# Mephisto405/WCMC

Measured on AMD Instinct MI355X. Metric: 128x128 MC patches/sec (train step), KPCN-Manifold, higher is better.
Workload: dtype bf16x321h

## Files before the change

### wcmc_amd/csrc/conv_bf16x3.hip

```cpp
#include <stdlib.h>

#include "common.h"
#include "conv_common.h"

namespace wcmc {

typedef __bf16 bf16x8 __attribute__((ext_vector_type(8)));
typedef unsigned short u16;
typedef short s16x4 __attribute__((ext_vector_type(4)));

__device__ __forceinline__ u16 f2bf(float x) { return __builtin_bit_cast(u16, (__bf16)x); }
__device__ __forceinline__ float bf2f(u16 h) { return __builtin_bit_cast(float, (unsigned)h << 16); }
__device__ __forceinline__ void split1(float x, u16& hi, u16& lo) {
  hi = f2bf(x);
  lo = f2bf(x - bf2f(hi));
}

__global__ void split_kernel(const float* __restrict__ x, int64_t xsn, int64_t xsh, int64_t xsw,
                             u16* __restrict__ out, int H, int W, int C, int Cp, int64_t total,
                             const float* __restrict__ post = nullptr, int64_t psn = 0, int64_t psh = 0, int64_t psw = 0,
                             int act = 0, float slope = 0.f) {
  const int V = Cp / 8;
  for (int64_t idx = (int64_t)blockIdx.x * blockDim.x + threadIdx.x; idx < total;
       idx += (int64_t)gridDim.x * blockDim.x) {
// ... 2372 lines not shown
  const int g = lane >> 4, li = lane & 15, tq = li >> 2, tp = li & 3;
  const int prow0 = wk * 32 + 4 * g + tq;
  auto tr_read = [&](const u16* base, int stride, int col0, bf16x8& out) {
    const u16* a0 = base + prow0 * stride + col0 + 4 * tp;
    const s16x4 lo4 = __builtin_amdgcn_ds_read_tr16_b64_v4i16(
        (s16x4 __attribute__((address_space(3)))*)(a0));
    const s16x4 hi4 = __builtin_amdgcn_ds_read_tr16_b64_v4i16(
        (s16x4 __attribute__((address_space(3)))*)(a0 + 16 * stride));
    typedef short s16x8 __attribute__((ext_vector_type(8)));
    const s16x8 cat = {lo4[0], lo4[1], lo4[2], lo4[3], hi4[0], hi4[1], hi4[2], hi4[3]};
    out = __builtin_bit_cast(bf16x8, cat);
  };

  if (nstages > 0) load_stage();
  for (int st = 0; st < nstages; ++st) {
    __syncthreads();
    store_stage();
    __syncthreads();
    if (st + 1 < nstages) load_stage();
    bf16x8 xh[4], xl[PL == 2 ? 4 : 1], yh[MT], yl[PL == 2 ? MT : 1];
#pragma unroll
    for (int j = 0; j < 4; ++j) {
      tr_read(Xs, SB, j * 16, xh[j]);
      if constexpr (PL == 2) tr_read(Xs + PK * SB, SB, j * 16, xl[j]);
    }
#pragma unroll
    for (int i = 0; i < MT; ++i) {
      tr_read(Ys, SA, (wm * MT + i) * 16, yh[i]);
      if constexpr (PL == 2) tr_read(Ys + PK * SA, SA, (wm * MT + i) * 16, yl[i]);
    }
    __builtin_amdgcn_sched_barrier(0);
#pragma unroll
    for (int i = 0; i < MT; ++i) {
      if (i < tm_valid) {
#pragma unroll
        for (int j = 0; j < 4; ++j) {
          if (j < tn_valid) {
            if constexpr (PL == 2) {
              acc[i][j] = __builtin_amdgcn_mfma_f32_16x16x32_bf16(yl[i], xh[j], acc[i][j], 0, 0, 0);
              acc[i][j] = __builtin_amdgcn_mfma_f32_16x16x32_bf16(yh[i], xl[j], acc[i][j], 0, 0, 0);
            }
            acc[i][j] = __builtin_amdgcn_mfma_f32_16x16x32_bf16(yh[i], xh[j], acc[i][j], 0, 0, 0);
          }
        }
      }
    }
  }
  __syncthreads();

  constexpr int RS = XC + 4;
  float* red = reinterpret_cast<float*>(smem16);
  const int fcol = lane & 15, fq = (lane >> 4) * 4;
  for (int h = 0; h < 2; ++h) {
    if (wk == h) {
#pragma unroll
      for (int i = 0; i < MT; ++i) {
        if (wm * MT + i < TM) {
#pragma unroll
          for (int j = 0; j < 4; ++j)
#pragma unroll
            for (int r = 0; r < 4; ++r) {
              float* q = red + ((wm * MT + i) * 16 + fq + r) * RS + j * 16 + fcol;
              *q = (h == 0 ? 0.f : *q) + acc[i][j][r];
            }
        }
      }
    }
    __syncthreads();
  }
  float* slab = p.slabs + ((int64_t)s * taps + tap) * p.Np * p.Cq;
  for (int idx = tid; idx < YC * (XC / 4); idx += 256) {
    const int r = idx / (XC / 4), c = (idx - r * (XC / 4)) * 4;
    if (co0 + r < p.Np && ci0 + c < p.Cq)
      *reinterpret_cast<float4*>(slab + (int64_t)(co0 + r) * p.Cq + ci0 + c) =
          *reinterpret_cast<const float4*>(red + r * RS + c);
  }
}


struct XWRowsParams {
  const u16* x; int N, H, W, Cpi;
  const u16* dy; int Ho, Wo, Cpo;
  int pad;
  float* slabs; int S, rps, R;
  float* dbg;
  int prio;
  int Np, Cq, coBlocks, ciBlocks;
  unsigned x_bytes, dy_bytes;
  int xps, yps;
};

constexpr int xwr_stride(int ch) { return ((ch / 16) | 1) * 16; }

struct XwrRaw { u32x2 a, b; };
template <int OFF2>
__device__ __forceinline__ void xwr_tr_issue(unsigned addr, XwrRaw& r) {
  asm volatile("ds_read_b64_tr_b16 %0, %2\n\tds_read_b64_tr_b16 %1, %2 offset:%3" : "=&v"(r.a), "=&v"(r.b) : "v"(addr), "n"(OFF2));
}
__device__ __forceinline__ bf16x8 xwr_cat(const XwrRaw& r) {
  const u32x4 c = {r.a[0], r.a[1], r.b[0], r.b[1]};
  return __builtin_bit_cast(bf16x8, c);
}

template <int OFF1, int OFF2>
__device__ __forceinline__ void xwr_tr_issue_at(unsigned addr, XwrRaw& r) {
  asm volatile("ds_read_b64_tr_b16 %0, %2 offset:%3\n\tds_read_b64_tr_b16 %1, %2 offset:%4"
               : "=&v"(r.a), "=&v"(r.b) : "v"(addr), "n"(OFF1), "n"(OFF2));
}

template <class F, int... I>
__device__ __forceinline__ void xstatic_for_impl(F&& f, std::integer_sequence<int, I...>) { (f(std::integral_constant<int, I>{}), ...); }
template <int N, class F>
__device__ __forceinline__ void xstatic_for(F&& f) { xstatic_for_impl(static_cast<F&&>(f), std::make_integer_sequence<int, N>{}); }

template <int KS, int TM, int NW, int DBG = 0, int PL = 2>
__global__ __launch_bounds__(NW * 64, (NW <= 4 ? 2 : 1)) void conv_wgrad_rows_bf16x3_kernel(XWRowsParams p) {
  constexpr int CHY = TM * 16, CHX = NW * 16, PK = 64, XR = PK + KS - 1;
  constexpr int SY = xwr_stride(CHY), SX = xwr_stride(CHX);
  constexpr int VY = SY / 8, VX = SX / 8;
  constexpr int YV = PK * VY, XV = XR * VX;
  constexpr int NVEC = PL * YV + PL * XV;
  constexpr int NI = (NVEC + NW * 64 - 1) / (NW * 64);
  constexpr int BUF = NI * NW * 64 * 8;
  extern __shared__ __attribute__((aligned(16))) u16 smem16[];

  const int tid = threadIdx.x, lane = tid & 63, wave = __builtin_amdgcn_readfirstlane(tid >> 6);
  const int xcd = blockIdx.x & 7, local = blockIdx.x >> 3;
  const int unit = (local / KS) * 8 + xcd;
  const int upb = p.coBlocks * p.ciBlocks;
  if (unit >= p.S * upb) return;
  const int trow = local % KS;
  const int s = unit / upb, ub = unit - s * upb;
  const int cob = ub / p.ciBlocks, cib = ub - cob * p.ciBlocks;
  const int co0 = cob * CHY, ci0 = cib * CHX;
  const int r0 = s * p.rps, r1 = min(p.R, r0 + p.rps);
  const int nch = (p.Wo + PK - 1) / PK;
  const int nrows = r1 - r0;
  const int nst = nrows * nch;

  const __amdgpu_buffer_rsrc_t xr = __builtin_amdgcn_make_buffer_rsrc((void*)p.x, 0, (int)p.x_bytes, 0x00020000);
  const __amdgpu_buffer_rsrc_t yr = __builtin_amdgcn_make_buffer_rsrc((void*)p.dy, 0, (int)p.dy_bytes, 0x00020000);

  unsigned relv[NI]; int rowv[NI];
#pragma unroll
  for (int i = 0; i < NI; ++i) {
    const int v = (i * NW + wave) * 64 + lane;
    unsigned rel = 0; int rw = 127;
    if (v < PL * YV) {
      const int plane = v >= YV, vv = v - plane * YV;
      const int row = vv / VY, vec = vv - row * VY;
      const int co = co0 + vec * 8;
      if (vec * 8 < CHY && co < p.Cpo) { rel = (unsigned)(row * p.yps + plane * 2 * p.Cpo + co * 2); rw = row; }
    } else if (v < NVEC) {
      const int u = v - PL * YV;
      const int plane = u >= XV, uu = u - plane * XV;
      const int row = uu / VX, vec = uu - row * VX;
      const int ci = ci0 + vec * 8;
      if (vec * 8 < CHX && ci < p.Cpi) { rel = (unsigned)(row * p.xps + plane * 2 * p.Cpi + ci * 2); rw = row; }
    }
    relv[i] = rel; rowv[i] = rw;
  }
  unsigned f_ybase = 0, f_xbase = 0, f_yn = 0, f_xn = 0; int f_xlo = 0, f_buf = 0;
  int f_c = 0, f_rs = nrows > 0 ? (nrows - trow % nrows) % nrows : 0, f_n, f_oy;
  const int f_n0 = r0 / p.Ho, f_oy0 = r0 - f_n0 * p.Ho;
  { const int r = r0 + f_rs; f_n = r / p.Ho; f_oy = r - f_n * p.Ho; }
  auto issue_prep = [&](int buf) {
// ... 475 lines not shown
                acc[q][i] = __builtin_amdgcn_mfma_f32_16x16x32_bf16(yh, xl[q], acc[q][i], 0, 0, 0);
              }
              acc[q][i] = __builtin_amdgcn_mfma_f32_16x16x32_bf16(yh, xh[q], acc[q][i], 0, 0, 0);
            }
            if (i == TM - 1 && kk + 1 < nk) {
              constexpr int K1 = 32 * SX * 2;
              XWR8_READ(K1, K1 + 16 * SX * 2, ax[q], rxh[q]);
              if constexpr (PL == 2) XWR8_READ(K1 + XLO, K1 + XLO + 16 * SX * 2, ax[q], rxl[q]);
            }
          }
          if (fill && kk * TM + i == 0) issue_prep(par ^ 1);
          if (fill && kk * TM + i < NI) issue_one(kk * TM + i);
          __builtin_amdgcn_sched_barrier(0);
        }
      }
    }
    if (fill) {
#pragma unroll
      for (int i = 0; i < NI; ++i)
        if (i >= nk * TM) issue_one(i);
    }
    cst(2);
  };
  for (int st = 0; st < nst; st += 2) {
    stage(st, std::integral_constant<int, 0>{});
    if (st + 1 < nst) stage(st + 1, std::integral_constant<int, 1>{});
  }
  rts(2);

  __syncthreads();
  constexpr int RS = CHX + 4;
  float* red = reinterpret_cast<float*>(smem16);
  const int fcol = lane & 15, fq = (lane >> 4) * 4;
  int etap[NS], eci[NS];
#pragma unroll
  for (int q = 0; q < NS; ++q) { const int pr = NS * wave + q; etap[q] = pr / NCI; eci[q] = pr - etap[q] * NCI; }
#pragma unroll
  for (int t = 0; t < KS; ++t) {
#pragma unroll
    for (int q = 0; q < NS; ++q)
      if (etap[q] == t) {
#pragma unroll
        for (int i = 0; i < TM; ++i)
#pragma unroll
          for (int r = 0; r < 4; ++r) red[(ycol[i] * 16 + fq + r) * RS + eci[q] * 16 + fcol] = acc[q][i][r];
      }
    if (XE) {
      if (t == ETAP) {
#pragma unroll
        for (int j = 0; j < NA; ++j)
          if (j < nex) {
#pragma unroll
            for (int r = 0; r < 4; ++r) red[(ycol[j] * 16 + fq + r) * RS + (ECI0 + epair) * 16 + fcol] = ace[j][r];
          }
      }
    } else if (t == ETAP && wave < TM) {
#pragma unroll
      for (int e = 0; e < NF; ++e)
#pragma unroll
        for (int r = 0; r < 4; ++r) red[(wave * 16 + fq + r) * RS + (ECI0 + e) * 16 + fcol] = ace[e][r];
    }
    __syncthreads();
    float* slab = p.slabs + (((int64_t)s * KS * KS + trow * KS + t) * p.Np + co0) * p.Cq + ci0;
    for (int idx = tid; idx < CHY * (CHX / 4); idx += NW * 64) {
      const int row = idx / (CHX / 4), v = idx - row * (CHX / 4);
      if (co0 + row < p.Np && ci0 + v * 4 < p.Cq)
        *reinterpret_cast<float4*>(slab + (int64_t)row * p.Cq + v * 4) = *reinterpret_cast<const float4*>(red + row * RS + v * 4);
    }
    __syncthreads();
  }
  if (DBG & 16) {
    asm volatile("s_waitcnt vmcnt(0)" ::: "memory");
    rts(3);
    if (lane == 0) {
      unsigned long long* o = reinterpret_cast<unsigned long long*>(p.dbg) + ((int64_t)blockIdx.x * NW + wave) * 8;
      for (int i = 0; i < 4; ++i) o[i] = rt[i];
      for (int i = 0; i < 3; ++i) o[4 + i] = cyc[i];
      o[7] = (unsigned long long)nst;
    }
  }
}
#undef XWR8_READ

template <int KS, int TM, int NW, int PL = 2>
static constexpr size_t xwr_lds_bytes() {
  constexpr int NVEC = PL * 64 * (xwr_stride(TM * 16) / 8) + PL * (64 + KS - 1) * (xwr_stride(NW * 16) / 8);
  constexpr int NI = (NVEC + NW * 64 - 1) / (NW * 64);
  constexpr size_t stage = (size_t)2 * NI * NW * 64 * 16;
  constexpr size_t red = (size_t)TM * 16 * (NW * 16 + 4) * sizeof(float);
  return stage > red ? stage : red;
}
static size_t xwr_lds_bytes_rt(int ks, int tm, int nw, int pl = 2) {
  const int nvec = pl * 64 * (xwr_stride(tm * 16) / 8) + pl * (64 + ks - 1) * (xwr_stride(nw * 16) / 8);
  const int ni = (nvec + nw * 64 - 1) / (nw * 64);
  const size_t stage = (size_t)2 * ni * nw * 64 * 16, red = (size_t)tm * 16 * (nw * 16 + 4) * sizeof(float);
  return stage > red ? stage : red;
}

template <int KS, int TM, int NW, int PL = 2>
static int launch_xwgrad_rows(const XWRowsParams& q, hipStream_t st) {
  constexpr size_t lds = xwr_lds_bytes<KS, TM, NW, PL>();
  const dim3 grid((unsigned)(((q.S * q.coBlocks * q.ciBlocks + 7) / 8) * 8 * KS));
  const char* r8e = ab_env("WCMC_WGRAD_ROWS8");
  const bool rows8 = r8e ? r8e[0] != '0' : PL == 2;
  if (KS == 5 && TM == 7 && NW == 7 && rows8) {
    constexpr size_t lds8 = (size_t)2 * ((PL * (64 * 14 + 68 * 14) + 511) / 512) * 512 * 16;
    if (PL == 1) {
      static LdsAttr attr81_set;
      if (set_max_lds(reinterpret_cast<const void*>(&conv_wgrad_rows8_bf16x3_kernel<0, 1, 1>), (size_t)lds8, attr81_set) != hipSuccess) return WCMC_ERR_LAUNCH;
      hipLaunchKernelGGL((conv_wgrad_rows8_bf16x3_kernel<0, 1, 1>), grid, dim3(512), lds8, st, q);
      return check_launch("conv2d_wgrad_bf16x3(rows8, one plane)");
    }
    static LdsAttr attr8_set, attr80_set;
#ifdef WCMC_DEBUG_BUILD
    { const char* e = ab_env("WCMC_DEBUG_ABLATE");
      const int ab = e ? atoi(e) : 0;
      auto kfn = ab == 16 ? &conv_wgrad_rows8_bf16x3_kernel<16> : ab == 1 ? &conv_wgrad_rows8_bf16x3_kernel<1> : ab == 2 ? &conv_wgrad_rows8_bf16x3_kernel<2>
                 : ab == 3 ? &conv_wgrad_rows8_bf16x3_kernel<3> : ab == 8 ? &conv_wgrad_rows8_bf16x3_kernel<8> : ab == 32 ? &conv_wgrad_rows8_bf16x3_kernel<32>
                 : ab == 34 ? &conv_wgrad_rows8_bf16x3_kernel<34> : ab == 35 ? &conv_wgrad_rows8_bf16x3_kernel<35> : nullptr;
      if (kfn) {
        (void)hipFuncSetAttribute(reinterpret_cast<const void*>(kfn), hipFuncAttributeMaxDynamicSharedMemorySize, (int)lds8);
        hipLaunchKernelGGL(kfn, grid, dim3(512), lds8, st, q);
        return check_launch("conv2d_wgrad_bf16x3(rows8 ablation / stamps)");
      } }
#endif
    if (set_max_lds(reinterpret_cast<const void*>(&conv_wgrad_rows8_bf16x3_kernel<0, 1>), (size_t)lds8, attr8_set) != hipSuccess) return WCMC_ERR_LAUNCH;
    if (set_max_lds(reinterpret_cast<const void*>(&conv_wgrad_rows8_bf16x3_kernel<0, 0>), (size_t)lds8, attr80_set) != hipSuccess) return WCMC_ERR_LAUNCH;
    if (x_env_on("WCMC_WGRAD_ROWS8_XE")) hipLaunchKernelGGL((conv_wgrad_rows8_bf16x3_kernel<0, 1>), grid, dim3(512), lds8, st, q);
    else hipLaunchKernelGGL((conv_wgrad_rows8_bf16x3_kernel<0, 0>), grid, dim3(512), lds8, st, q);
    return check_launch("conv2d_wgrad_bf16x3(rows8)");
  }
#ifdef WCMC_DEBUG_BUILD
  if (KS == 5 && TM == 7 && NW == 7 && PL == 2) {
    int ab;
    { const char* e = ab_env("WCMC_DEBUG_ABLATE"); ab = e ? atoi(e) : 0; }
    if (ab == 1 || ab == 2 || ab == 3 || ab == 4 || ab == 8 || ab == 16) {
      auto kfn = ab == 16 ? &conv_wgrad_rows_bf16x3_kernel<5, 7, 7, 16> : ab == 1 ? &conv_wgrad_rows_bf16x3_kernel<5, 7, 7, 1> : ab == 2 ? &conv_wgrad_rows_bf16x3_kernel<5, 7, 7, 2>
                 : ab == 3 ? &conv_wgrad_rows_bf16x3_kernel<5, 7, 7, 3> : ab == 4 ? &conv_wgrad_rows_bf16x3_kernel<5, 7, 7, 4>
                 : &conv_wgrad_rows_bf16x3_kernel<5, 7, 7, 8>;
      (void)hipFuncSetAttribute(reinterpret_cast<const void*>(kfn), hipFuncAttributeMaxDynamicSharedMemorySize, (int)lds);
      hipLaunchKernelGGL(kfn, grid, dim3(448), lds, st, q);
      return check_launch("conv2d_wgrad_bf16x3(rows ablation)");
    }
  }
#endif
  static LdsAttr attr_set;
  if (set_max_lds(reinterpret_cast<const void*>(&conv_wgrad_rows_bf16x3_kernel<KS, TM, NW, 0, PL>), (size_t)lds, attr_set) != hipSuccess) return WCMC_ERR_LAUNCH;
  hipLaunchKernelGGL((conv_wgrad_rows_bf16x3_kernel<KS, TM, NW, 0, PL>), grid, dim3(NW * 64), lds, st, q);
  return check_launch("conv2d_wgrad_bf16x3(rows)");
}

__global__ __launch_bounds__(256) void colsum_split_kernel(const u16* __restrict__ dy, int Cp, int C, int64_t M,
                                                            int64_t per_block, float* __restrict__ partial) {
  extern __shared__ __attribute__((aligned(16))) float smem[];
  const int V = Cp / 8;
  const int PL = 256 / V;
  const int v = threadIdx.x % V, pl = threadIdx.x / V;
  const int64_t p0 = (int64_t)blockIdx.x * per_block, p1 = min(M, p0 + per_block);
  float acc[8] = {0.f, 0.f, 0.f, 0.f, 0.f, 0.f, 0.f, 0.f};
  if (pl < PL) {
    for (int64_t q = p0 + pl; q < p1; q += PL) {
      const u16* r = dy + q * 2 * Cp + v * 8;
      const uint4 h = *reinterpret_cast<const uint4*>(r), l = *reinterpret_cast<const uint4*>(r + Cp);
      const unsigned hw[4] = {h.x, h.y, h.z, h.w}, lw[4] = {l.x, l.y, l.z, l.w};
#pragma unroll
      for (int e = 0; e < 4; ++e) {
        acc[2 * e] += __builtin_bit_cast(float, hw[e] << 16) + __builtin_bit_cast(float, lw[e] << 16);
        acc[2 * e + 1] += __builtin_bit_cast(float, hw[e] & 0xffff0000u) + __builtin_bit_cast(float, lw[e] & 0xffff0000u);
      }
    }
#pragma unroll
    for (int e = 0; e < 8; ++e) smem[(pl * V + v) * 8 + e] = acc[e];
  }
  __syncthreads();
  if (pl == 0) {
    for (int q = 1; q < PL; ++q)
#pragma unroll
      for (int e = 0; e < 8; ++e) acc[e] += smem[(q * V + v) * 8 + e];
#pragma unroll
    for (int e = 0; e < 8; ++e)
      if (v * 8 + e < C) partial[(int64_t)blockIdx.x * C + v * 8 + e] = acc[e];
  }
}

static int x_pick_nt(int tiles) {
  const int cand[4] = {7, 4, 2, 1};
  int best = 1, best_cost = 1 << 30;
  for (int i = 0; i < 4; ++i) {
    const int nt = cand[i];
    const int cost = ((tiles + nt - 1) / nt) * (nt + 2);
    if (cost < best_cost) { best_cost = cost; best = nt; }
  }
  return best;
}

struct XWgradPlan { int rows, rps, R, rTM, rNW; int TM, coBlocks, ciBlocks, S, Np, Cq, G; int64_t pix_per_split, per_block; size_t slab_elems, bytes; };
static XWgradPlan x_plan_wgrad(int N, int Ho, int Wo, int Cout, int Cin, int ks, int terms = 3) {
  XWgradPlan pl;
  pl.Np = round_up(Cout, 16); pl.Cq = round_up(Cin, 16);
  const int coT = pl.Np / 16, ciT = pl.Cq / 16;
  pl.TM = (coT % 7 == 0) ? 7 : 4;
  pl.coBlocks = (coT + pl.TM - 1) / pl.TM;
  pl.ciBlocks = (ciT + 3) / 4;
  const int64_t M = (int64_t)N * Ho * Wo;
  const int taps = ks * ks;
  const int rows_on = x_env_on("WCMC_WGRAD_ROWS");
  pl.R = N * Ho; pl.rps = 0; pl.rows = 0; pl.rTM = pl.rNW = 0;
  if (rows_on && (ks == 5 || ks == 3 || (ks == 1 && x_env_on("WCMC_WGRAD_ROWS_1X1"))) && (int64_t)N * Ho >= 64) {
    int tm = 0, nw = 0;
    if (ks == 5) { tm = coT % 7 == 0 ? 7 : 0; nw = ciT % 7 == 0 ? 7 : ciT == 3 ? 3 : 0; }
    else if (ks == 1) {
      if (coT == 8 && ciT == 8) { tm = 8; nw = 8; }
    }
    else if (ks == 3) {
      const int wide = x_env_on("WCMC_WGRAD_ROWS_3X3");
      const char* e44 = ab_env("WCMC_WGRAD_44");
      if (coT % 8 == 0 && ciT % 8 == 0 && (ciT >= 16 || wide) && !(e44 && e44[0] == '1')) { tm = 8; nw = 8; }
      else if (wide && coT % 4 == 0 && ciT % 4 == 0) { tm = 4; nw = 4; }
    }
    if (tm && nw) {
      pl.rows = 1; pl.rTM = tm; pl.rNW = nw;
      pl.coBlocks = coT / tm; pl.ciBlocks = ciT / nw;
      const size_t lds = xwr_lds_bytes_rt(ks, tm, nw, terms == 1 ? 1 : 2);
      int wpc = (int)((160 * 1024) / lds);
      int wcap = nw <= 4 ? 2 : 1;
// ... 666 lines not shown
  p.mask_out = (unsigned char*)mask1;
  p.ks = 1; p.pad = 0; p.act = act1; p.slope = slope1;
  p.Kp = p.Cpi; p.Kt = round_up(p.Cpi, 32); p.Np = round_up(Cout1, 16);
  p.CS = p.Kp; p.nslabs = 1; p.SPS = p.Kt / 32; p.PXS = 0; p.CSl = p.CS; p.SPSl = p.SPS; p.ap = 2; p.wplanes = 2; p.f16 = 0;
  p.tilesY = p.tilesX = 0; p.G = x_colsum_rows(N, H, W); p.colsum = colsum1;
  p.M = (int64_t)N * H * W;
  const int cp2 = round_up(Cout2, 4);
  const int64_t xb = p.M * 4 * p.Cpi, yb = p.M * 4 * p.Np;
  const int64_t y2b = ((int64_t)(N - 1) * y2sn + (int64_t)(H - 1) * y2sh + (int64_t)(W - 1) * y2sw + cp2) * 4;
  WCMC_REQUIRE(xb < 0x7ff00000LL && yb < 0x7ff00000LL && y2b < 0x7ff00000LL && y2sn >= 0 && y2sh >= 0 && y2sw >= cp2,
               WCMC_ERR_BAD_ARG, "conv1x1_pair_bf16x3: operand larger than 2 GiB (split the batch)");
  p.x_bytes = (unsigned)xb; p.wp_bytes = (unsigned)((size_t)p.Np * 2 * p.Kt * sizeof(u16));
  p.y_bytes = (unsigned)yb; p.m_bytes = (unsigned)(p.M * (p.Np / 8));
  p.wp2 = (const u16*)wp2; p.bias2 = bias2; p.y2 = y2; p.y2sn = y2sn; p.y2sh = y2sh; p.y2sw = y2sw;
  p.Cout2 = Cout2; p.act2 = act2; p.slope2 = slope2; p.Kt2 = p.Np;
  p.wp2_bytes = (unsigned)((size_t)round_up(Cout2, 16) * 2 * p.Kt2 * sizeof(u16)); p.y2_bytes = (unsigned)y2b;
  hipStream_t st = (hipStream_t)stream;
  if (kind == 1) return launch_xpw2<8, 32, true, 1>(p, st);
  if (kind == 2) return launch_xpw2<8, 2, true, 2>(p, st);
  return launch_xpw2<4, 16, true, 2>(p, st);
}

extern "C" size_t wcmc_conv2d_igemm_colsum_elems(int N, int Ho, int Wo, int Cout) {
  if (N <= 0 || Ho <= 0 || Wo <= 0 || Cout <= 0) return 0;
  return (size_t)x_colsum_rows(N, Ho, Wo) * round_up(Cout, 16) + 4;
}

extern "C" int wcmc_colsum_finish(const float* partial, int N, int Ho, int Wo, int Cout, float* db, void* stream) {
  WCMC_REQUIRE(partial && db && N > 0 && Ho > 0 && Wo > 0 && Cout > 0, WCMC_ERR_BAD_ARG, "colsum_finish: bad argument");
  const int G = x_colsum_rows(N, Ho, Wo), Np = round_up(Cout, 16);
  hipLaunchKernelGGL(colsum_final_strided_kernel, dim3((unsigned)((Cout + 63) / 64)), dim3(1024), 0,
                     (hipStream_t)stream, partial, G, Np, Cout, db);
  return check_launch("colsum_finish");
}

extern "C" size_t wcmc_conv2d_wgrad_bf16x3_workspace_bytes(int N, int Ho, int Wo, int Cout, int Cin, int ks) {
  if (N <= 0 || Ho <= 0 || Wo <= 0 || Cout <= 0 || Cin <= 0 || ks <= 0) return 0;
  const size_t b3 = x_plan_wgrad(N, Ho, Wo, Cout, Cin, ks, 3).bytes, b1 = x_plan_wgrad(N, Ho, Wo, Cout, Cin, ks, 1).bytes;
  return b3 > b1 ? b3 : b1;
}

template <int TM, int PL = 2>
static int launch_xwgrad(const XWgradParams& p, hipStream_t stream) {
  constexpr size_t lds_stage = (size_t)PL * 64 * (xw_stride(TM * 16) + xw_stride(64)) * sizeof(u16);
  constexpr size_t lds_red = (size_t)TM * 16 * (64 + 4) * sizeof(float);
  constexpr size_t lds = lds_stage > lds_red ? lds_stage : lds_red;
  const int per_split = p.ks * p.ks * p.coBlocks * p.ciBlocks;
  const dim3 grid((unsigned)(((p.S + 7) / 8) * 8 * per_split));
  hipLaunchKernelGGL((conv_wgrad_bf16x3_kernel<TM, PL>), grid, dim3(256), lds, stream, p);
  return check_launch("conv2d_wgrad_bf16x3");
}

extern "C" int wcmc_conv2d_wgrad_bf16x3(const void* x_split, int N, int H, int W, int Cin, const void* dy_split,
                                        int Cout, int ks, int pad, float* dw, float* db, void* workspace,
                                        size_t workspace_bytes, int phase, const float* dy_colsum_partial, int terms,
                                        void* stream) {
  WCMC_REQUIRE(N > 0 && H > 0 && W > 0 && Cin > 0 && Cout > 0 && ks > 0 && pad >= 0 && dw && workspace &&
                   x_split && dy_split,
               WCMC_ERR_BAD_ARG, "conv2d_wgrad_bf16x3: bad argument");
  WCMC_REQUIRE(terms == 3 || terms == 1, WCMC_ERR_BAD_ARG,
               "conv2d_wgrad_bf16x3: terms must be 3 (hi*hi + hi*lo + lo*hi) or 1 (the hi planes only)");
  const int Ho = H + 2 * pad - ks + 1, Wo = W + 2 * pad - ks + 1;
  WCMC_REQUIRE(Ho > 0 && Wo > 0, WCMC_ERR_BAD_ARG, "conv2d_wgrad_bf16x3: empty output");
  WCMC_REQUIRE(aligned16(x_split) && aligned16(dy_split), WCMC_ERR_ALIGNMENT,
               "conv2d_wgrad_bf16x3: split buffers must be 16-byte aligned");
  const XWgradPlan pl = x_plan_wgrad(N, Ho, Wo, Cout, Cin, ks, terms);
  WCMC_REQUIRE(workspace_bytes >= pl.bytes && aligned16(workspace), WCMC_ERR_WORKSPACE,
               "conv2d_wgrad_bf16x3: workspace %zu < %zu bytes (or unaligned)", workspace_bytes, pl.bytes);
  hipStream_t st = (hipStream_t)stream;
  XWgradParams p;
  p.x = (const u16*)x_split; p.N = N; p.H = H; p.W = W; p.Cin = Cin; p.Cpi = round_up(Cin, 8);
  p.dy = (const u16*)dy_split; p.Ho = Ho; p.Wo = Wo; p.Cout = Cout; p.Cpo = round_up(Cout, 8);
  p.ks = ks; p.pad = pad; p.slabs = (float*)workspace; p.S = pl.S; p.M = (int64_t)N * Ho * Wo;
  p.pix_per_split = pl.pix_per_split; p.Np = pl.Np; p.Cq = pl.Cq; p.coBlocks = pl.coBlocks; p.ciBlocks = pl.ciBlocks;
  const size_t xb = wcmc_split_elems(N, H, W, Cin) * sizeof(u16), yb = wcmc_split_elems(N, Ho, Wo, Cout) * sizeof(u16);
  WCMC_REQUIRE(xb < 0x7ff00000u && yb < 0x7ff00000u, WCMC_ERR_BAD_ARG,
               "conv2d_wgrad_bf16x3: operand larger than 2 GiB (split the batch)");
  p.x_bytes = (unsigned)xb; p.dy_bytes = (unsigned)yb;
  p.xps = 4 * p.Cpi; p.yps = 4 * p.Cpo;
  WCMC_REQUIRE(phase >= 0 && phase <= 2, WCMC_ERR_BAD_ARG, "conv2d_wgrad_bf16x3: phase must be 0, 1 or 2");
  int rc = 0;
  if (phase != 2 && pl.rows) {
    XWRowsParams q;
    q.x = p.x; q.N = N; q.H = H; q.W = W; q.Cpi = p.Cpi; q.dy = p.dy; q.Ho = Ho; q.Wo = Wo; q.Cpo = p.Cpo;
    q.dbg = (float*)workspace + pl.slab_elems;
    { const char* e = ab_env("WCMC_WGRAD_ROWS8_PRIO"); q.prio = e ? atoi(e) : 8; if (q.prio < 0 || q.prio > 13) q.prio = 0; }
    q.pad = pad; q.slabs = p.slabs; q.S = pl.S; q.rps = pl.rps; q.R = pl.R; q.Np = pl.Np; q.Cq = pl.Cq;
    q.coBlocks = pl.coBlocks; q.ciBlocks = pl.ciBlocks; q.x_bytes = p.x_bytes; q.dy_bytes = p.dy_bytes;
    q.xps = p.xps; q.yps = p.yps;
    const int key = (terms == 1 ? 1000 : 0) + ks * 100 + pl.rTM * 10 + pl.rNW;
    switch (key) {
      case 577: rc = launch_xwgrad_rows<5, 7, 7>(q, st); break;
      case 573: rc = launch_xwgrad_rows<5, 7, 3>(q, st); break;
      case 388: rc = launch_xwgrad_rows<3, 8, 8>(q, st); break;
      case 344: rc = launch_xwgrad_rows<3, 4, 4>(q, st); break;
      case 188: rc = launch_xwgrad_rows<1, 8, 8>(q, st); break;
      case 1577: rc = launch_xwgrad_rows<5, 7, 7, 1>(q, st); break;
      case 1573: rc = launch_xwgrad_rows<5, 7, 3, 1>(q, st); break;
      case 1388: rc = launch_xwgrad_rows<3, 8, 8, 1>(q, st); break;
      case 1344: rc = launch_xwgrad_rows<3, 4, 4, 1>(q, st); break;
      case 1188: rc = launch_xwgrad_rows<1, 8, 8, 1>(q, st); break;
      default: WCMC_REQUIRE(false, WCMC_ERR_BAD_ARG, "conv2d_wgrad_bf16x3: no filter-row instance for the plan");
    }
  } else if (phase != 2) {
    if (terms == 1) rc = pl.TM == 7 ? launch_xwgrad<7, 1>(p, st) : launch_xwgrad<4, 1>(p, st);
    else rc = pl.TM == 7 ? launch_xwgrad<7>(p, st) : launch_xwgrad<4>(p, st);
  }
  if (rc || phase == 1) return rc;
  const bool fuse_db = db && dy_colsum_partial;
  const int cs_rows = fuse_db ? (Cout + 63) / 64 : 0;
  size_t red_lds = (size_t)WR_CI * (ks * ks + 1) * sizeof(float) + 256 * sizeof(float);
  if (fuse_db && red_lds < (size_t)16 * 64 * sizeof(float)) red_lds = (size_t)16 * 64 * sizeof(float);
  hipLaunchKernelGGL(wgrad_reduce_kernel, dim3((unsigned)((Cin + WR_CI - 1) / WR_CI), (unsigned)(Cout + cs_rows)), dim3(256),
                     red_lds, st, p.slabs, dw, pl.S, ks * ks, Cout, Cin, pl.Np, pl.Cq, fuse_db ? dy_colsum_partial : nullptr,
                     x_colsum_rows(N, Ho, Wo), round_up(Cout, 16), db);
  rc = check_launch("conv2d_wgrad_bf16x3_reduce");
  if (rc || !db || fuse_db) return rc;
  float* partial = (float*)workspace + pl.slab_elems;
  WCMC_REQUIRE(p.Cpo / 8 <= 256, WCMC_ERR_BAD_ARG, "conv2d_wgrad_bf16x3: Cout > 2048 unsupported");
  hipLaunchKernelGGL(colsum_split_kernel, dim3((unsigned)pl.G), dim3(256), (size_t)256 * 8 * sizeof(float), st, p.dy,
                     p.Cpo, Cout, p.M, pl.per_block, partial);
  hipLaunchKernelGGL(colsum_final_kernel, dim3((unsigned)((Cout + 63) / 64)), dim3(1024), 0, st, partial, pl.G, Cout,
                     db);
  return check_launch("conv2d_bias_grad_bf16x3");
}
```

Baseline: 724.1.

## Add packed 8-wave wgrad kernel for ~100-channel 5x5 single-plane convs

Adds a new 5x5 weight-gradient kernel for the single-plane (terms==1) path when Cin is 97..100 and fits one ci block. It uses 8 waves that each own 4 (tap, ci-block) pairs. Six full 16-channel column blocks per tap are computed densely, and the 4-channel remainder of all five taps is packed into two shared MFMA tiles, so padded channels no longer waste matrix work. It keeps the LDS DMA ring and transposed ds_read pipelining, and on by default it replaces the previous rows8 one-plane kernel for these shapes. The cost is more complex reduction and scatter logic for the packed tiles, plus a new kernel variant with an env opt-out.

Result: faster. 735.3 (median of 6 runs) (+1.5%).

```diff
diff --git a/wcmc_amd/csrc/conv_bf16x3.hip b/wcmc_amd/csrc/conv_bf16x3.hip
--- a/wcmc_amd/csrc/conv_bf16x3.hip
+++ b/wcmc_amd/csrc/conv_bf16x3.hip
@@ -2478,6 +2478,7 @@
   const u16* x; int N, H, W, Cpi;
   const u16* dy; int Ho, Wo, Cpo;
   int pad;
+  int Cin;
   float* slabs; int S, rps, R;
   float* dbg;
   int prio;
@@ -3119,6 +3120,288 @@
 }
 #undef XWR8_READ
 
+template <int DBG = 0, int NB = 2>
+__global__ __launch_bounds__(512, 1) void conv_wgrad_rows8p_bf16x3_kernel(XWRowsParams p) {
+  constexpr int KS = 5, TM = 7, NCI = 7, NCF = 6, NW = 8, NS = 4;
+  constexpr int CHY = TM * 16, CHX = NCI * 16, PK = 64, XR = PK + KS - 1;
+  constexpr int SY = xwr_stride(CHY), SX = xwr_stride(CHX);
+  constexpr int VY = SY / 8, VX = SX / 8;
+  constexpr int YV = PK * VY, XV = XR * VX;
+  constexpr int NVEC = YV + XV;
+  constexpr int NI = (NVEC + NW * 64 - 1) / (NW * 64);
+  constexpr int BUF = NI * NW * 64 * 8;
+  constexpr int NSET = (NB + 1) / 2;
+  static_assert(NB >= 2 && NB <= 4 && NCF * KS + 2 == NS * NW, "32 pairs over 8 waves");
+  static_assert(BUF * 2 + (32 + 16) * SX * 2 + 64 < 65536 && BUF * 2 + (32 + 16) * SY * 2 + TM * 32 < 65536, "ds_read offset field");
+  extern __shared__ __attribute__((aligned(16))) u16 smem16[];
+
+  const int tid = threadIdx.x, lane = tid & 63, wave = __builtin_amdgcn_readfirstlane(tid >> 6);
+  const int xcd = blockIdx.x & 7, local = blockIdx.x >> 3;
+  const int unit = (local / KS) * 8 + xcd;
+  const int upb = p.coBlocks * p.ciBlocks;
+  if (unit >= p.S * upb) return;
+  const int trow = local % KS;
+  const int s = unit / upb, ub = unit - s * upb;
+  const int cob = ub / p.ciBlocks, cib = ub - cob * p.ciBlocks;
+  const int co0 = cob * CHY, ci0 = cib * CHX;
+  const int r0 = s * p.rps, r1 = min(p.R, r0 + p.rps);
+  const int nch = (p.Wo + PK - 1) / PK;
+  const int nrows = r1 - r0;
+  const int nst = nrows * nch;
+
+  const __amdgpu_buffer_rsrc_t xr = __builtin_amdgcn_make_buffer_rsrc((void*)p.x, 0, (int)p.x_bytes, 0x00020000);
+  const __amdgpu_buffer_rsrc_t yr = __builtin_amdgcn_make_buffer_rsrc((void*)p.dy, 0, (int)p.dy_bytes, 0x00020000);
+
+  unsigned relv[NI]; int rowv[NI];
+#pragma unroll
+  for (int i = 0; i < NI; ++i) {
+    const int v = (i * NW + wave) * 64 + lane;
+    unsigned rel = 0; int rw = 127;
+    if (v < YV) {
+      const int row = v / VY, vec = v - row * VY;
+      const int co = co0 + vec * 8;
+      if (vec * 8 < CHY && co < p.Cpo) { rel = (unsigned)(row * p.yps + co * 2); rw = row; }
+    } else if (v < NVEC) {
+      const int u = v - YV;
+      const int row = u / VX, vec = u - row * VX;
+      const int ci = ci0 + vec * 8;
+      if (vec * 8 < CHX && ci < p.Cpi) { rel = (unsigned)(row * p.xps + ci * 2); rw = row; }
+    }
+    relv[i] = rel; rowv[i] = rw;
+  }
+  unsigned f_ybase = 0, f_xbase = 0, f_yn = 0, f_xn = 0; int f_xlo = 0, f_buf = 0;
+  int f_c = 0, f_rs = nrows > 0 ? (nrows - trow % nrows) % nrows : 0, f_n, f_oy;
+  const int f_n0 = r0 / p.Ho, f_oy0 = r0 - f_n0 * p.Ho;
+  { const int r = r0 + f_rs; f_n = r / p.Ho; f_oy = r - f_n * p.Ho; }
+  auto issue_prep = [&](int buf) {
+    const int ox0 = f_c * PK;
+    const int iy = f_oy + trow - p.pad;
+    const bool rowok = (unsigned)iy < (unsigned)p.H;
+    f_ybase = (unsigned)(((f_n * p.Ho + f_oy) * p.Wo + ox0) * p.yps);
+    f_xbase = (unsigned)(((f_n * p.H + iy) * p.W + ox0 - p.pad) * p.xps);
+    f_yn = (unsigned)max(0, p.Wo - ox0);
+    f_xlo = p.pad - ox0;
+    f_xn = rowok ? (unsigned)p.W : 0u;
+    f_buf = buf;
+    if (++f_c == nch) {
+      f_c = 0;
+      if (++f_rs == nrows) { f_rs = 0; f_n = f_n0; f_oy = f_oy0; }
+      else if (++f_oy == p.Ho) { f_oy = 0; ++f_n; }
+    }
+  };
+  const bool short_wave = ((NI - 1) * NW + wave) * 64 >= NVEC;
+  auto issue_one = [&](int i) {
+    if (i == NI - 1 && short_wave) return;
+    const bool isx = (i * NW + NW - 1) * 64 < YV ? false : i * NW * 64 >= YV ? true : (i * NW + wave) * 64 >= YV;
+    const unsigned base = isx ? f_xbase : f_ybase, cnt = isx ? f_xn : f_yn;
+    const int lo = isx ? f_xlo : 0;
+    const unsigned off = (unsigned)(rowv[i] - lo) < cnt ? base + relv[i] : XOOB;
+    __attribute__((address_space(3))) void* dst =
+        (__attribute__((address_space(3))) void*)(smem16 + f_buf * BUF + (i * NW + wave) * 512);
+    if (!isx) __builtin_amdgcn_raw_ptr_buffer_load_lds(yr, dst, 16, off, 0, 0, 0);
+    else __builtin_amdgcn_raw_ptr_buffer_load_lds(xr, dst, 16, off, 0, 0, 0);
+  };
+  auto dma_wait = [&](int k) {
+    const int n = k * (short_wave ? NI - 1 : NI);
+    static_assert(NI == 4, "the counts below");
+    switch (n) {
+      case 3: asm volatile("s_waitcnt vmcnt(3)" ::: "memory"); break;
+      case 4: asm volatile("s_waitcnt vmcnt(4)" ::: "memory"); break;
+      case 6: asm volatile("s_waitcnt vmcnt(6)" ::: "memory"); break;
+      case 8: asm volatile("s_waitcnt vmcnt(8)" ::: "memory"); break;
+      default: asm volatile("s_waitcnt vmcnt(0)" ::: "memory"); break;
+    }
+  };
+
+  f32x4 acc[NS][TM];
+#pragma unroll
+  for (int q = 0; q < NS; ++q)
+#pragma unroll
+    for (int i = 0; i < TM; ++i) acc[q][i] = f32x4{0.f, 0.f, 0.f, 0.f};
+
+  const int g = lane >> 4, li = lane & 15, tq = li >> 2, tp = li & 3;
+  const unsigned lds0 = (unsigned)(uintptr_t)((__attribute__((address_space(3))) u16*)smem16);
+
+  unsigned long long rt[4] = {0, 0, 0, 0}, cyc[3] = {0, 0, 0}, tprev = 0;
+  auto rts = [&](int i) {
+    if (DBG & 16) {
+      unsigned long long t;
+      __builtin_amdgcn_sched_barrier(0);
+      asm volatile("s_memrealtime %0\n\ts_waitcnt lgkmcnt(0)" : "=s"(t)::"memory");
+      __builtin_amdgcn_sched_barrier(0);
+      rt[i] = t;
+    }
+  };
+  auto cst = [&](int i) {
+    if (DBG & 16) {
+      unsigned long long t;
+      __builtin_amdgcn_sched_barrier(0);
+      asm volatile("s_memtime %0\n\ts_waitcnt lgkmcnt(0)" : "=s"(t)::"memory");
+      __builtin_amdgcn_sched_barrier(0);
+      if (i >= 0) cyc[i] += t - tprev;
+      tprev = t;
+    }
+  };
+  rts(0);
+#pragma unroll
+  for (int b = 0; b < NB - 1; ++b)
+    if (b < nst) {
+      issue_prep(b);
+#pragma unroll
+      for (int i = 0; i < NI; ++i) issue_one(i);
+    }
+  rts(1);
+  cst(-1);
+  unsigned ayv[NSET], axv[NSET][NS];
+  {
+    const int prow0 = 4 * g + tq;
+#pragma unroll
+    for (int ss = 0; ss < NSET; ++ss) {
+      ayv[ss] = lds0 + (unsigned)((2 * ss * BUF + prow0 * SY + 4 * tp) * 2); asm volatile("" : "+v"(ayv[ss]));
+      const int xb = 2 * ss * BUF + PK * SY;
+#pragma unroll
+      for (int q = 0; q < NS; ++q) {
+        const int pr = NS * wave + q, pt = pr / NCF, pc = pr - pt * NCF;
+        const int full = xb + (prow0 + pt) * SX + pc * 16 + 4 * tp;
+        const int pack = xb + (prow0 + tp + (pr - NCF * KS)) * SX + NCF * 16;
+        axv[ss][q] = lds0 + (unsigned)((pr < NCF * KS ? full : pack) * 2); asm volatile("" : "+v"(axv[ss][q]));
+      }
+    }
+  }
+  auto stage = [&](const int st, auto PAR) __attribute__((always_inline)) {
+    constexpr int par = decltype(PAR)::value, BO = (par & 1) * BUF * 2;
+    { int k = nst - 1 - st; if (k > NB - 2) k = NB - 2; dma_wait(k); }
+    asm volatile("s_waitcnt lgkmcnt(0)" ::: "memory");
+    __builtin_amdgcn_s_barrier();
+    cst(0);
+    const bool fill = st + NB - 1 < nst;
+    cst(1);
+    if (p.prio) { if (wave < 4) __builtin_amdgcn_s_setprio(2); else __builtin_amdgcn_s_setprio(1); }
+    const unsigned ay = ayv[par >> 1];
+    const unsigned (&ax)[NS] = axv[par >> 1];
+    const int c = st % nch;
+    const int nk = (min(PK, p.Wo - c * PK) + 31) / 32;
+    constexpr int PF = 1;
+    static_assert(NS == 4 && (PF == 1 || PF == 2), "lgkmcnt(10) below = the next dy fragment + 2 NS reads of x");
+    XwrRaw rx[NS], ry[PF + 1];
+#pragma unroll
+    for (int q = 0; q < NS; ++q) xwr_tr_issue_at<BO, BO + 16 * SX * 2>(ax[q], rx[q]);
+    xwr_tr_issue_at<BO, BO + 16 * SY * 2>(ay, ry[0]);
+    if constexpr (PF == 2) xwr_tr_issue_at<BO + 32, BO + 32 + 16 * SY * 2>(ay, ry[1]);
+    bf16x8 xh[NS];
+    xstatic_for<2>([&](auto K_) {
+      constexpr int kk = decltype(K_)::value;
+      if (kk < nk) {
+        xstatic_for<TM>([&](auto I_) {
+          constexpr int i = decltype(I_)::value;
+          constexpr int j = kk * TM + i, cur = j % (PF + 1), nxt = (j + PF) % (PF + 1);
+          constexpr int KY = 32 * SY * 2;
+          if (j > 0 && p.prio == j && wave < 4) __builtin_amdgcn_s_setprio(0);
+          if constexpr (PF == 1) asm volatile("s_waitcnt lgkmcnt(0)" : "+v"(ry[cur].a), "+v"(ry[cur].b));
+          else if (i + 1 < TM || kk + 1 < nk) {
+            if (i == TM - 1) asm volatile("s_waitcnt lgkmcnt(10)" : "+v"(ry[cur].a), "+v"(ry[cur].b));
+            else asm volatile("s_waitcnt lgkmcnt(2)" : "+v"(ry[cur].a), "+v"(ry[cur].b));
+          } else asm volatile("s_waitcnt lgkmcnt(0)" : "+v"(ry[cur].a), "+v"(ry[cur].b));
+          if (i == 0) {
+#pragma unroll
+            for (int q = 0; q < NS; ++q) { asm volatile("" : "+v"(rx[q].a), "+v"(rx[q].b)); xh[q] = xwr_cat(rx[q]); }
+          }
+          const bf16x8 yh = xwr_cat(ry[cur]);
+          if constexpr (i + PF < TM) {
+            constexpr int O = BO + kk * KY + (i + PF) * 32;
+            xwr_tr_issue_at<O, O + 16 * SY * 2>(ay, ry[nxt]);
+          } else if (kk + 1 < nk) {
+            constexpr int O = BO + (kk + 1) * KY + (i + PF - TM) * 32;
+            xwr_tr_issue_at<O, O + 16 * SY * 2>(ay, ry[nxt]);
+          }
+          __builtin_amdgcn_sched_barrier(0);
+#pragma unroll
+          for (int q = 0; q < NS; ++q) {
+            if (DBG & 1) { asm volatile("" ::"v"(yh), "v"(xh[q])); }
+            else acc[q][i] = __builtin_amdgcn_mfma_f32_16x16x32_bf16(yh, xh[q], acc[q][i], 0, 0, 0);
+            if (i == TM - PF && kk + 1 < nk) {
+              constexpr int K1 = BO + 32 * SX * 2;
+              xwr_tr_issue_at<K1, K1 + 16 * SX * 2>(ax[q], rx[q]);
+            }
+          }
+          if (fill && j == 0) issue_prep((par + NB - 1) % NB);
+          if (fill && j < NI) issue_one(j);
+          __builtin_amdgcn_sched_barrier(0);
+        });
+      }
+    });
+    if (fill) {
+#pragma unroll
+      for (int i = 0; i < NI; ++i)
+        if (i >= nk * TM) issue_one(i);
+    }
+    cst(2);
+  };
+  for (int st = 0; st < nst; st += NB) {
+    xstatic_for<NB>([&](auto P_) {
+      constexpr int par = decltype(P_)::value;
+      if (par == 0 || st + par < nst) stage(st + par, P_);
+    });
+  }
+  rts(2);
+
+  __syncthreads();
+  constexpr int RS = CHX + 4;
+  float* red = reinterpret_cast<float*>(smem16);
+  const int fcol = lane & 15, fq = (lane >> 4) * 4;
+#pragma unroll
+  for (int t = 0; t < KS; ++t) {
+#pragma unroll
+    for (int q = 0; q < NS; ++q) {
+      const int pr = NS * wave + q;
+      if (pr < NCF * KS) {
+        if (pr / NCF == t) {
+          const int pc = pr - t * NCF;
+#pragma unroll
+          for (int i = 0; i < TM; ++i)
+#pragma unroll
+            for (int r = 0; r < 4; ++r) red[(i * 16 + fq + r) * RS + pc * 16 + fcol] = acc[q][i][r];
+        }
+      } else if (pr == NCF * KS) {
+        if (t == 0) {
+#pragma unroll
+          for (int i = 0; i < TM; ++i)
+#pragma unroll
+            for (int r = 0; r < 4; ++r) red[(i * 16 + fq + r) * RS + NCF * 16 + fcol] = fcol < 4 ? acc[q][i][r] : 0.f;
+        } else if (t < 4 && (fcol >> 2) == t) {
+#pragma unroll
+          for (int i = 0; i < TM; ++i)
+#pragma unroll
+            for (int r = 0; r < 4; ++r) red[(i * 16 + fq + r) * RS + NCF * 16 + (fcol & 3)] = acc[q][i][r];
+        }
+      } else if (t == 4 && (fcol >> 2) == 3) {
+#pragma unroll
+        for (int i = 0; i < TM; ++i)
+#pragma unroll
+          for (int r = 0; r < 4; ++r) red[(i * 16 + fq + r) * RS + NCF * 16 + (fcol & 3)] = acc[q][i][r];
+      }
+    }
+    __syncthreads();
+    float* slab = p.slabs + (((int64_t)s * KS * KS + trow * KS + t) * p.Np + co0) * p.Cq + ci0;
+    for (int idx = tid; idx < CHY * (CHX / 4); idx += NW * 64) {
+      const int row = idx / (CHX / 4), v = idx - row * (CHX / 4);
+      if (co0 + row < p.Np && ci0 + v * 4 < p.Cq)
+        *reinterpret_cast<float4*>(slab + (int64_t)row * p.Cq + v * 4) = *reinterpret_cast<const float4*>(red + row * RS + v * 4);
+    }
+    __syncthreads();
+  }
+  if (DBG & 16) {
+    asm volatile("s_waitcnt vmcnt(0)" ::: "memory");
+    rts(3);
+    if (lane == 0) {
+      unsigned long long* o = reinterpret_cast<unsigned long long*>(p.dbg) + ((int64_t)blockIdx.x * NW + wave) * 8;
+      for (int i = 0; i < 4; ++i) o[i] = rt[i];
+      for (int i = 0; i < 3; ++i) o[4 + i] = cyc[i];
+      o[7] = (unsigned long long)nst;
+    }
+  }
+}
+
 template <int KS, int TM, int NW, int PL = 2>
 static constexpr size_t xwr_lds_bytes() {
   constexpr int NVEC = PL * 64 * (xwr_stride(TM * 16) / 8) + PL * (64 + KS - 1) * (xwr_stride(NW * 16) / 8);
@@ -3140,10 +3423,42 @@
   const dim3 grid((unsigned)(((q.S * q.coBlocks * q.ciBlocks + 7) / 8) * 8 * KS));
   const char* r8e = ab_env("WCMC_WGRAD_ROWS8");
   const bool rows8 = r8e ? r8e[0] != '0' : PL == 2;
+  if (KS == 5 && TM == 7 && NW == 7 && PL == 1 && !r8e && q.ciBlocks == 1 && q.Cin > 96 && q.Cin <= 100) {
+    const char* pe = ab_env("WCMC_WGRAD_PACKED");
+    if (!(pe && pe[0] == '0')) {
+      constexpr size_t buf8p = (size_t)((64 * 14 + 68 * 14 + 511) / 512) * 512 * 16;
+      static LdsAttr attrp2_set;
+#ifdef WCMC_DEBUG_BUILD
+      { const char* e = ab_env("WCMC_DEBUG_ABLATE"); const char* re = ab_env("WCMC_WGRAD_RING");
+        const int ab = e ? atoi(e) : 0, ring = re ? atoi(re) : 2;
+        auto kfn = ring == 3 ? (ab == 16 ? &conv_wgrad_rows8p_bf16x3_kernel<16, 3> : &conv_wgrad_rows8p_bf16x3_kernel<0, 3>)
+                   : ring == 4 ? (ab == 16 ? &conv_wgrad_rows8p_bf16x3_kernel<16, 4> : &conv_wgrad_rows8p_bf16x3_kernel<0, 4>)
+                   : ab == 16 ? &conv_wgrad_rows8p_bf16x3_kernel<16, 2> : ab == 1 ? &conv_wgrad_rows8p_bf16x3_kernel<1, 2> : nullptr;
+        if (kfn) {
+          const size_t ldsp = (ring == 3 ? 3 : ring == 4 ? 4 : 2) * buf8p;
+          (void)hipFuncSetAttribute(reinterpret_cast<const void*>(kfn), hipFuncAttributeMaxDynamicSharedMemorySize, (int)ldsp);
+          hipLaunchKernelGGL(kfn, grid, dim3(512), ldsp, st, q);
+          return check_launch("conv2d_wgrad_bf16x3(rows8p, debug instance)");
+        } }
+#endif
+      if (set_max_lds(reinterpret_cast<const void*>(&conv_wgrad_rows8p_bf16x3_kernel<0, 2>), 2 * buf8p, attrp2_set) != hipSuccess) return WCMC_ERR_LAUNCH;
+      hipLaunchKernelGGL((conv_wgrad_rows8p_bf16x3_kernel<0, 2>), grid, dim3(512), 2 * buf8p, st, q);
+      return check_launch("conv2d_wgrad_bf16x3(rows8p)");
+    }
+  }
   if (KS == 5 && TM == 7 && NW == 7 && rows8) {
     constexpr size_t lds8 = (size_t)2 * ((PL * (64 * 14 + 68 * 14) + 511) / 512) * 512 * 16;
     if (PL == 1) {
       static LdsAttr attr81_set;
+#ifdef WCMC_DEBUG_BUILD
+      { const char* e = ab_env("WCMC_DEBUG_ABLATE");
+        if (e && atoi(e) == 16) {
+          auto kfn = &conv_wgrad_rows8_bf16x3_kernel<16, 1, 1>;
+          (void)hipFuncSetAttribute(reinterpret_cast<const void*>(kfn), hipFuncAttributeMaxDynamicSharedMemorySize, (int)lds8);
+          hipLaunchKernelGGL(kfn, grid, dim3(512), lds8, st, q);
+          return check_launch("conv2d_wgrad_bf16x3(rows8, one plane, stamps)");
+        } }
+#endif
       if (set_max_lds(reinterpret_cast<const void*>(&conv_wgrad_rows8_bf16x3_kernel<0, 1, 1>), (size_t)lds8, attr81_set) != hipSuccess) return WCMC_ERR_LAUNCH;
       hipLaunchKernelGGL((conv_wgrad_rows8_bf16x3_kernel<0, 1, 1>), grid, dim3(512), lds8, st, q);
       return check_launch("conv2d_wgrad_bf16x3(rows8, one plane)");
@@ -3178,6 +3493,15 @@
       (void)hipFuncSetAttribute(reinterpret_cast<const void*>(kfn), hipFuncAttributeMaxDynamicSharedMemorySize, (int)lds);
       hipLaunchKernelGGL(kfn, grid, dim3(448), lds, st, q);
       return check_launch("conv2d_wgrad_bf16x3(rows ablation)");
+    }
+  }
+  if (KS == 5 && TM == 7 && NW == 7 && PL == 1) {
+    const char* e = ab_env("WCMC_DEBUG_ABLATE");
+    if (e && atoi(e) == 16) {
+      auto kfn = &conv_wgrad_rows_bf16x3_kernel<5, 7, 7, 16, 1>;
+      (void)hipFuncSetAttribute(reinterpret_cast<const void*>(kfn), hipFuncAttributeMaxDynamicSharedMemorySize, (int)lds);
+      hipLaunchKernelGGL(kfn, grid, dim3(448), lds, st, q);
+      return check_launch("conv2d_wgrad_bf16x3(rows, one plane, stamps)");
     }
   }
 #endif
@@ -4010,7 +4334,7 @@
   int rc = 0;
   if (phase != 2 && pl.rows) {
     XWRowsParams q;
-    q.x = p.x; q.N = N; q.H = H; q.W = W; q.Cpi = p.Cpi; q.dy = p.dy; q.Ho = Ho; q.Wo = Wo; q.Cpo = p.Cpo;
+    q.x = p.x; q.N = N; q.H = H; q.W = W; q.Cpi = p.Cpi; q.Cin = Cin; q.dy = p.dy; q.Ho = Ho; q.Wo = Wo; q.Cpo = p.Cpo;
     q.dbg = (float*)workspace + pl.slab_elems;
     { const char* e = ab_env("WCMC_WGRAD_ROWS8_PRIO"); q.prio = e ? atoi(e) : 8; if (q.prio < 0 || q.prio > 13) q.prio = 0; }
     q.pad = pad; q.slabs = p.slabs; q.S = pl.S; q.rps = pl.rps; q.R = pl.R; q.Np = pl.Np; q.Cq = pl.Cq;
```
